# qq456cvb/CPPF2

Hardware: AMD Instinct MI355X
Metric: scenes/sec (1/2/4/8 GPU) at 4096 pts x 20k tuples; 5deg5cm match vs ref (higher is better)
Workload: dtype f32

## Files before the change

cppf2_amd/csrc/cppf_backvote.hip:

```cpp
#include "cppf_common.h"


template <typename KeyFn>
__device__ uint32_t radix_select_keys(KeyFn key, int n, int kth, uint32_t* s_hist , int* s_misc ,
                                      int* n_le) {
  uint32_t prefix = 0;
  int remaining = kth;
  int below = 0;
  const int shifts[3] = {21, 10, 0};
  const int widths[3] = {11, 11, 10};
  uint32_t mask_fixed = 0;
  for (int pass = 0; pass < 3; ++pass) {
    const int sh = shifts[pass], nbins = 1 << widths[pass];
    for (int i = threadIdx.x; i < nbins; i += blockDim.x) s_hist[i] = 0;
    __syncthreads();
    for (int i = threadIdx.x; i < n; i += blockDim.x) {
      const uint32_t bits = key(i);
      if ((bits & mask_fixed) == prefix) atomicAdd(&s_hist[(bits >> sh) & (nbins - 1)], 1u);
    }
    __syncthreads();
    if (threadIdx.x < 64) {
      const int per = nbins / 64;
      uint32_t sum = 0;
      for (int j = 0; j < per; ++j) sum += s_hist[threadIdx.x * per + j];
      uint32_t incl = sum;
#pragma unroll
      for (int off = 1; off < 64; off <<= 1) {
        const uint32_t o = __shfl_up(incl, off);
        if ((int)threadIdx.x >= off) incl += o;
      }
      const uint32_t excl = incl - sum;
      if ((uint32_t)remaining >= excl && (uint32_t)remaining < incl) {
        uint32_t run = excl;
        for (int j = 0; j < per; ++j) {
          const uint32_t c = s_hist[threadIdx.x * per + j];
          if ((uint32_t)remaining < run + c) {
            s_misc[0] = threadIdx.x * per + j;
            s_misc[1] = (int)run;
            s_misc[2] = (int)c;
            break;
          }
          run += c;
        }
      }
    }
    __syncthreads();
    const int bin = s_misc[0];
    below += s_misc[1];
    remaining -= s_misc[1];
    prefix |= ((uint32_t)bin) << sh;
    mask_fixed |= ((uint32_t)(nbins - 1)) << sh;
    if (pass == 2) *n_le = below + s_misc[2];
    __syncthreads();
  }
  return prefix;
}

__device__ uint32_t radix_select(const float* __restrict__ v, int n, int kth, uint32_t* s_hist, int* s_misc,
                                 int* n_le) {
  return radix_select_keys([v](int i) { return __float_as_uint(v[i]); }, n, kth, s_hist, s_misc, n_le);
}

__device__ __forceinline__ uint32_t float_key(float f) {
  const uint32_t u = __float_as_uint(f);
  return (u & 0x80000000u) ? ~u : (u | 0x80000000u);
}
__device__ __forceinline__ float key_float(uint32_t k) {
  return __uint_as_float((k & 0x80000000u) ? (k & 0x7fffffffu) : ~k);
}

__global__ __launch_bounds__(256) void backvote_errs_kernel(const float* __restrict__ pts,
                                                            const int32_t* __restrict__ pt_off,
                                                            const int32_t* __restrict__ idx, int k,
                                                            const int32_t* __restrict__ tup_off,
                                                            const float* __restrict__ tr,
                                                            const double* __restrict__ centers, Axes9 axes,
                                                            float* __restrict__ errs) {
  const int b = blockIdx.y;
  const float* p = pts + 3 * (int64_t)pt_off[b];
  const int t0 = tup_off[b], nt = tup_off[b + 1] - t0;
  const double cx = centers[3 * b], cy = centers[3 * b + 1], cz = centers[3 * b + 2];
  for (int t = blockIdx.x * 256 + threadIdx.x; t < nt; t += gridDim.x * 256) {
    const int64_t row = (int64_t)(t0 + t);
    const float* a = p + 3 * (int64_t)idx[row * k];
    const float* bb = p + 3 * (int64_t)idx[row * k + 1];
    float tb[2];
    target_pair(a[0], a[1], a[2], bb[0], bb[1], bb[2], cx, cy, cz, axes.a, tb, nullptr);
    const float d0 = tr[row * 2] - tb[0], d1 = tr[row * 2 + 1] - tb[1];
    errs[row] = __builtin_sqrtf(d0 * d0 + d1 * d1);
  }
}

__global__ __launch_bounds__(BV_THREADS) void backvote_kernel(
    const float* __restrict__ pts, const int32_t* __restrict__ pt_off, const int32_t* __restrict__ idx, int k,
    const int32_t* __restrict__ tup_off, const float* __restrict__ tr, const double* __restrict__ centers,
    Axes9 axes, const int32_t* __restrict__ kidx, const float* __restrict__ gammas, double margin, int num_rots,
    uint8_t* __restrict__ mask, int32_t* __restrict__ kept_tuple, int32_t* __restrict__ kept_count,
    double* __restrict__ kept_wt, int32_t* __restrict__ kept_row0, float* __restrict__ errs,
    float* __restrict__ thr_out, int32_t* __restrict__ hits) {
  __shared__ uint32_t s_hist[2048];
  __shared__ int s_misc[4];
  __shared__ int s_wave[BV_THREADS / 64];
  __shared__ float s_f[BV_THREADS / 64];
  const int b = blockIdx.x;
  const int p0 = pt_off[b];
  const float* p = pts + 3 * (int64_t)p0;
  const int t0 = tup_off[b], nt = tup_off[b + 1] - t0;
  float* e = errs + t0;
  if (nt <= 0) {
    if (threadIdx.x == 0) { kept_count[b] = 0; if (thr_out) thr_out[b] = NAN; }
    return;
  }
  int kq = kidx[b];
  if (kq > nt - 1) kq = nt - 1;
  const float gamma = gammas[b];
  int n_le = 0;
  const uint32_t bits_lo = radix_select(e, nt, kq, s_hist, s_misc, &n_le);
  const float v_lo = __uint_as_float(bits_lo);
  float v_hi = v_lo;
  if (kq + 1 <= nt - 1 && kq + 1 >= n_le) {
    uint32_t mn = 0xffffffffu;
    for (int i = threadIdx.x; i < nt; i += BV_THREADS) {
      const uint32_t bits = __float_as_uint(e[i]);
      if (bits > bits_lo && bits < mn) mn = bits;
    }
#pragma unroll
    for (int off = 32; off > 0; off >>= 1) mn = min(mn, (uint32_t)__shfl_xor((int)mn, off));
    if (wave_lane() == 0) s_hist[threadIdx.x >> 6] = mn;
    __syncthreads();
    if (threadIdx.x == 0) {
      for (int w = 1; w < BV_THREADS / 64; ++w) mn = min(mn, s_hist[w]);
      s_hist[64] = mn;
    }
    __syncthreads();
    v_hi = __uint_as_float(s_hist[64]);
    __syncthreads();
  }
  const float diff = v_hi - v_lo;
  float thr = v_lo + diff * gamma;
  if (gamma >= 0.5f) thr = v_hi - diff * (1.0f - gamma);
  if (threadIdx.x == 0 && thr_out) thr_out[b] = thr;
  int kept = 0;
  for (int base = 0; base < nt; base += BV_THREADS) {
    const int t = base + threadIdx.x;
    const bool keep = (t < nt) && (e[t] < thr);
    if (t < nt) mask[t0 + t] = keep ? 1 : 0;
    int tot;
    const int pos = block_scan_flag(keep, s_wave, &tot);
    if (keep) kept_tuple[t0 + kept + pos] = t;
    kept += tot;
  }
  if (threadIdx.x == 0) kept_count[b] = kept;
  __syncthreads();
  int32_t* h = hits + p0;
  for (int j = threadIdx.x; j < kept; j += BV_THREADS) {
    const int64_t row = (int64_t)(t0 + kept_tuple[t0 + j]);
    atomicAdd(&h[idx[row * k]], 1);
    atomicAdd(&h[idx[row * k + 1]], 1);
  }
  __threadfence();
  __syncthreads();
  int hmax = 0;
  for (int j = threadIdx.x; j < kept; j += BV_THREADS) {
    const int64_t row = (int64_t)(t0 + kept_tuple[t0 + j]);
    hmax = max(hmax, __hip_atomic_load(&h[idx[row * k]], __ATOMIC_RELAXED, __HIP_MEMORY_SCOPE_AGENT));
    hmax = max(hmax, __hip_atomic_load(&h[idx[row * k + 1]], __ATOMIC_RELAXED, __HIP_MEMORY_SCOPE_AGENT));
  }
#pragma unroll
  for (int off = 32; off > 0; off >>= 1) hmax = max(hmax, __shfl_xor(hmax, off));
  if (wave_lane() == 0) s_wave[threadIdx.x >> 6] = hmax;
  __syncthreads();
  hmax = 0;
  for (int w = 0; w < BV_THREADS / 64; ++w) hmax = max(hmax, s_wave[w]);
  __syncthreads();
  const double dmax = (double)hmax;
  int rank = 0;
  for (int base = 0; base < kept; base += BV_THREADS) {
    const int j = base + threadIdx.x;
    bool valid = false;
    if (j < kept) {
      const int64_t row = (int64_t)(t0 + kept_tuple[t0 + j]);
      const int i0 = idx[row * k], i1 = idx[row * k + 1];
      const double w0 = (double)__hip_atomic_load(&h[i0], __ATOMIC_RELAXED, __HIP_MEMORY_SCOPE_AGENT) / dmax;
      const double w1 = (double)__hip_atomic_load(&h[i1], __ATOMIC_RELAXED, __HIP_MEMORY_SCOPE_AGENT) / dmax;
      kept_wt[t0 + j] = (w0 + w1) + margin;
      const float dx = p[3 * i0] - p[3 * i1], dy = p[3 * i0 + 1] - p[3 * i1 + 1], dz = p[3 * i0 + 2] - p[3 * i1 + 2];
      valid = norm3_fused(dx, dy, dz) > 1e-7f;
    }
    int tot;
    const int pos = block_scan_flag(valid, s_wave, &tot);
    if (j < kept) kept_row0[t0 + j] = valid ? (rank + pos) * num_rots : -1;
    rank += tot;
  }
  (void)s_f;
}

extern "C" int64_t cppf_backvote_workspace_bytes(int64_t total_points, int B) {
  (void)B;
  return align_up(total_points * 4, 256);
}

extern "C" int cppf_backvote_filter(int B, const float* pts, const int32_t* pt_off, const int32_t* idx, int k,
                                    const int32_t* tup_off, const float* tr, const double* centers,
                                    const double* h_axes, const int32_t* kidx, const float* gammas,
                                    double imp_wt_margin, int num_rots, uint8_t* mask, int32_t* kept_tuple,
                                    int32_t* kept_count, double* kept_wt, int32_t* kept_row0, float* back_errs,
                                    float* thr, void* workspace, int64_t workspace_bytes, void* stream) {
  CPPF_CHECK_ARG(B > 0 && pts && pt_off && idx && tup_off && tr && centers && h_axes && kidx && gammas);
  CPPF_CHECK_ARG(mask && kept_tuple && kept_count && kept_wt && kept_row0 && back_errs);
  CPPF_CHECK_ARG(workspace && workspace_bytes > 0);
  Axes9 ax;
  for (int i = 0; i < 9; ++i) ax.a[i] = h_axes[i];
  CPPF_HIP(hipMemsetAsync(workspace, 0, (size_t)workspace_bytes, (hipStream_t)stream));
  hipLaunchKernelGGL(backvote_errs_kernel, dim3(B >= 32 ? 16 : 64, B), dim3(256), 0, (hipStream_t)stream, pts, pt_off,
                     idx, k, tup_off, tr, centers, ax, back_errs);
  CPPF_LAUNCH_CHECK();
  hipLaunchKernelGGL(backvote_kernel, dim3(B), dim3(BV_THREADS), 0, (hipStream_t)stream, pts, pt_off, idx, k, tup_off,
                     tr, centers, ax, kidx, gammas, imp_wt_margin, num_rots, mask, kept_tuple, kept_count, kept_wt,
                     kept_row0, back_errs, thr, (int32_t*)workspace);
  CPPF_LAUNCH_CHECK();
  return CPPF_OK;
}

#define ASM_STAGE 4096
__global__ __launch_bounds__(256) void assemble_pose_kernel(
    const float* __restrict__ sphere, const int32_t* __restrict__ up_idx, const float* __restrict__ up_count,
    const int32_t* __restrict__ right_idx, const float* __restrict__ right_count, int up_axis, int right_axis,
    const int64_t* __restrict__ argmax, const uint32_t* __restrict__ peak, const double* __restrict__ world,
    const CppfSceneGrid* __restrict__ grids, const float* __restrict__ pred_scales,
    const int32_t* __restrict__ tup_off, const int32_t* __restrict__ kept_tuple,
    const int32_t* __restrict__ kept_count, CppfSceneResult* __restrict__ out) {
  const int b = blockIdx.x;
  __shared__ float s_med[3];
  const int kept = kept_count ? kept_count[b] : 0;
  if (threadIdx.x < 3) s_med[threadIdx.x] = NAN;
  __syncthreads();
  if (pred_scales && kept > 0) {
    __shared__ uint32_t s_hist[2048];
    __shared__ int s_misc[4];
    const int t0 = tup_off[b];
    const int target = (kept - 1) / 2;
    __shared__ uint32_t s_keys[3][ASM_STAGE];
    const bool staged = kept <= ASM_STAGE;
    if (staged) {
      for (int i = threadIdx.x; i < kept; i += blockDim.x) {
        const float* row = pred_scales + (int64_t)(t0 + kept_tuple[t0 + i]) * 3;
        s_keys[0][i] = float_key(row[0]); s_keys[1][i] = float_key(row[1]); s_keys[2][i] = float_key(row[2]);
      }
      __syncthreads();
    }
    for (int col = 0; col < 3; ++col) {
      int n_le;
      uint32_t k;
      if (staged) {
        const uint32_t* keys = s_keys[col];
        k = radix_select_keys([=](int i) { return keys[i]; }, kept, target, s_hist, s_misc, &n_le);
      } else {
        k = radix_select_keys(
            [=](int i) { return float_key(pred_scales[(int64_t)(t0 + kept_tuple[t0 + i]) * 3 + col]); }, kept, target,
            s_hist, s_misc, &n_le);
      }
      if (threadIdx.x == 0) s_med[col] = key_float(k);
    }
  }
  __syncthreads();
  if (threadIdx.x != 0) return;
  CppfSceneResult r;
  r.argmax = argmax[b];
  r.peak = peak ? peak[b] : 0u;
  r.t[0] = world[3 * b]; r.t[1] = world[3 * b + 1]; r.t[2] = world[3 * b + 2];
  r.up_idx = up_idx[b]; r.right_idx = right_idx[b];
  r.up_count = up_count ? up_count[b] : 0.0f;
  r.right_count = right_count ? right_count[b] : 0.0f;
  r.kept = kept;
  r.flags = (grids ? grids[b].flags : 0) | ((peak && peak[b] == 0xFFFFFFFFu) ? 4 : 0);
  r.ncell = grids ? grids[b].ncell : 0;
  r.pad_[0] = r.pad_[1] = r.pad_[2] = 0;
  r.scale[0] = s_med[0]; r.scale[1] = s_med[1]; r.scale[2] = s_med[2];
  pose_from_bins(sphere, r.up_idx, r.right_idx, up_axis, right_axis, r.R);
  out[b] = r;
}

extern "C" int cppf_assemble_pose(int B, const float* sphere, const int32_t* up_idx, const float* up_count,
                                  const int32_t* right_idx, const float* right_count, int up_axis, int right_axis,
                                  const int64_t* argmax, const uint32_t* peak, const double* world,
                                  const CppfSceneGrid* grids, const float* pred_scales, const int32_t* tup_off,
                                  const int32_t* kept_tuple, const int32_t* kept_count, CppfSceneResult* out,
                                  void* stream) {
  CPPF_CHECK_ARG(B > 0 && sphere && up_idx && right_idx && argmax && world && out);
  CPPF_CHECK_ARG(up_axis >= 0 && up_axis < 3 && right_axis >= 0 && right_axis < 3 && up_axis != right_axis);
  CPPF_CHECK_ARG(pred_scales == nullptr || (tup_off && kept_tuple && kept_count));
  hipLaunchKernelGGL(assemble_pose_kernel, dim3(B), dim3(256), 0, (hipStream_t)stream, sphere, up_idx, up_count,
                     right_idx, right_count, up_axis, right_axis, argmax, peak, world, grids, pred_scales, tup_off,
                     kept_tuple, kept_count, out);
  CPPF_LAUNCH_CHECK();
  return CPPF_OK;
}

// ... 36 lines not shown
```

cppf2_amd/csrc/cppf_mlp_split.hip:

```cpp
#include "cppf_common.h"
#include <atomic>
#include <type_traits>

typedef float f32x16 __attribute__((ext_vector_type(16)));
typedef float f32x4 __attribute__((ext_vector_type(4)));
typedef __bf16 bf16x8 __attribute__((ext_vector_type(8)));

__host__ __device__ constexpr int rs_waves(int nt) { return nt >= 6 ? 4 : 8; }
#define RS_RESLAYER 0
#define RS_LINEAR 1
#define RS_SUMGATHER 2
#define RS_ENCODE 3
#define RS_SUMENCODE 5
__host__ __device__ constexpr int rs_waves_mode(int nt, int mode) { return mode == RS_LINEAR ? 8 : rs_waves(nt); }
#define RS_STAGE_TILES 16
#define RS_FRAG_BYTES 1024
__host__ __device__ constexpr int rs_stage_bytes(int stg) { return stg * 3 * RS_FRAG_BYTES; }
__host__ __device__ constexpr int rs_tile_bytes(int pc) { return pc * RS_FRAG_BYTES; }

#ifndef RS_DBG
#define RS_DBG 0
#endif
typedef unsigned u32x4 __attribute__((ext_vector_type(4)));
typedef float f32x2 __attribute__((ext_vector_type(2)));
// ... 229 lines not shown
  constexpr int SPC = rs_spc(NTILES, Stream::STG_);
  float xv[8];
  RS_WAIT(4, 15);
  __builtin_amdgcn_sched_barrier(0);
  xs.read(xv, 0, 0);
  RsFrag b = rs_split<PC>(xv);
  int slot = 1;
  bool whole = true;
  for (int s0 = 0; s0 < ks1; s0 += SPC) {
    const u32x4* w = (s0 > 0 && whole) ? ws.template acquire<2 * (SPC - 1)>() : ws.template acquire<0>();
    whole = s0 + SPC <= ks1;
#pragma unroll
    for (int i = 0; i < SPC; ++i) {
      if (s0 + i < ks1) {
        RS_WAIT(2, 15);
        __builtin_amdgcn_sched_barrier(0);
        xs.read(xv, s0 + i + 1, slot);
        xs.issue(s0 + i + 3, slot == 0 ? 2 : slot - 1, rw);
        slot = slot == 2 ? 0 : slot + 1;
        RsFrag bn;
        rs_step<NTILES, Stream::PMAX, PC>(acc, w + i * NTILES * PC * 64, b,
                        [&](int p) { rs_split_pair<PC, true>(xv[2 * p], xv[2 * p + 1], bn.h[p], bn.m[p], bn.l[p]); },
                        [&](int q) { if (i == 0) ws.piece(q); });
        b = bn;
      }
    }
  }
}

template <int NS, int NTILES, int PC, class Stream>
__device__ __forceinline__ void rs_product_h(f32x16 (&dst)[NTILES], const f32x16 (&src)[NS], Stream& ws, float bs) {
  constexpr int SPC = rs_spc(NTILES, Stream::STG_);
  static_assert((2 * NS) % SPC == 0, "whole chunks");
  RsFrag b;
#pragma unroll
  for (int p = 0; p < 4; ++p)
    rs_split_pair<PC>(PC == 2 ? src[0][2 * p] * bs : src[0][2 * p], PC == 2 ? src[0][2 * p + 1] * bs : src[0][2 * p + 1], b.h[p], b.m[p], b.l[p]);
#pragma unroll
  for (int c = 0; c < 2 * NS / SPC; ++c) {
    const u32x4* w = ws.template acquire<0>();
#pragma unroll
    for (int i = 0; i < SPC; ++i) {
      const int step = c * SPC + i, nx = (step + 1 < 2 * NS) ? step + 1 : step;
      RsFrag bn = b;
      rs_step<NTILES, Stream::PMAX, PC>(dst, w + i * NTILES * PC * 64, b,
                      [&](int p) {
                        if (step + 1 < 2 * NS) {
                          const float s0 = src[nx >> 1][8 * (nx & 1) + 2 * p], s1 = src[nx >> 1][8 * (nx & 1) + 2 * p + 1];
                          rs_split_pair<PC, true>(PC == 2 ? s0 * bs : s0, PC == 2 ? s1 * bs : s1, bn.h[p], bn.m[p], bn.l[p]);
                        }
                      },
                      [&](int q) { if (i == 0) ws.piece(q); });
      b = bn;
    }
  }
}

__device__ __forceinline__ float rs_relu(float h) { return __builtin_elementwise_maximum(h, 0.0f); }

__device__ __forceinline__ void rs_load_tile(f32x16& acc, const float* v, int g) {
#pragma unroll
  for (int q = 0; q < 4; ++q) {
    const f32x4 t = *reinterpret_cast<const f32x4*>(v + 8 * q + 4 * g);
    acc[4 * q + 0] = t.x; acc[4 * q + 1] = t.y; acc[4 * q + 2] = t.z; acc[4 * q + 3] = t.w;
  }
}

__device__ __forceinline__ void rs_load_tile_scaled(f32x16& acc, const float* v, int g, float sc) {
#pragma unroll
  for (int q = 0; q < 4; ++q) {
    const f32x4 t = *reinterpret_cast<const f32x4*>(v + 8 * q + 4 * g);
    acc[4 * q + 0] = t.x * sc; acc[4 * q + 1] = t.y * sc; acc[4 * q + 2] = t.z * sc; acc[4 * q + 3] = t.w * sc;
  }
}

struct RsDecode {
  const float* prior = nullptr;
  const float* prior_pos = nullptr;
  float prior_inv_sigma = 0.0f;
  const float* uniforms = nullptr;
  int32_t* bins = nullptr;
};

template <int NT, int PC>
__device__ __forceinline__ void rs_decode_epilogue(f32x16 (&o)[NT], const RsDecode& dc, int64_t row, bool in, int g, float bs) {
  static_assert(NT == 6, "6 coordinates x 32 bins");
  if (PC == 2) {
#pragma unroll
    for (int u = 0; u < 6; ++u) o[u] *= bs;
  }
  if (dc.prior) {
    const float* pr = dc.prior + row * 192 + 4 * g;
#pragma unroll
    for (int u = 0; u < 6; ++u) {
#pragma unroll
      for (int q = 0; q < 4; ++q) {
        const f32x4 v = *reinterpret_cast<const f32x4*>(pr + 32 * u + 8 * q);
        o[u][4 * q + 0] += v.x; o[u][4 * q + 1] += v.y; o[u][4 * q + 2] += v.z; o[u][4 * q + 3] += v.w;
      }
    }
  } else if (dc.prior_pos) {
    const float* pp = dc.prior_pos + row * 6;
    const float is = dc.prior_inv_sigma;
#pragma unroll
    for (int u = 0; u < 6; ++u) {
      const float pos = pp[u];
#pragma unroll
      for (int e = 0; e < 16; ++e) {
        const float z = ((float)((e & 3) + 8 * (e >> 2) + 4 * g) - pos) * is;
        o[u][e] += (z * z) * -0.5f;
      }
    }
  }
  float back[6], tot[6];
#pragma unroll
  for (int u = 0; u < 6; ++u) {
    float m = o[u][0];
#pragma unroll
    for (int e = 1; e < 16; ++e) m = fmaxf(m, o[u][e]);
    m = fmaxf(m, __shfl_xor(m, 32));
#pragma unroll
    for (int e = 0; e < 16; ++e) o[u][e] = softmax_exp(o[u][e] - m);
    back[u] = 0.0f;
  }
#pragma unroll
  for (int q = 0; q < 4; ++q) {
    float ta[6][4], tb[6][4], fwd[6];
#pragma unroll
    for (int u = 0; u < 6; ++u) {
      ta[u][0] = back[u] + o[u][4 * q + 0];
      ta[u][1] = ta[u][0] + o[u][4 * q + 1];
      ta[u][2] = ta[u][1] + o[u][4 * q + 2];
      ta[u][3] = ta[u][2] + o[u][4 * q + 3];
    }
#pragma unroll
    for (int u = 0; u < 6; ++u) fwd[u] = __shfl_xor(ta[u][3], 32);
#pragma unroll
    for (int u = 0; u < 6; ++u) {
      tb[u][0] = fwd[u] + o[u][4 * q + 0];
      tb[u][1] = tb[u][0] + o[u][4 * q + 1];
      tb[u][2] = tb[u][1] + o[u][4 * q + 2];
      tb[u][3] = tb[u][2] + o[u][4 * q + 3];
    }
#pragma unroll
    for (int u = 0; u < 6; ++u) {
      back[u] = __shfl_xor(tb[u][3], 32);
      tot[u] = g ? tb[u][3] : back[u];
#pragma unroll
      for (int i = 0; i < 4; ++i) o[u][4 * q + i] = g ? tb[u][i] : ta[u][i];
    }
  }
  const float* ur = dc.uniforms + row * 6;
#pragma unroll
  for (int u = 0; u < 6; ++u) {
    const float target = ur[u] * tot[u];
    int cnt = 0;
#pragma unroll
    for (int e = 0; e < 16; ++e) cnt += (o[u][e] <= target) ? 1 : 0;
    cnt += __shfl_xor(cnt, 32);
    if (in && g == 0) dc.bins[row * 6 + u] = cnt < 31 ? cnt : 31;
  }
}

__device__ __forceinline__ void rs_claim_store(int* p, int v) { __hip_atomic_store(p, v, __ATOMIC_RELAXED, __HIP_MEMORY_SCOPE_WORKGROUP); }
__device__ __forceinline__ int rs_claim_load(int* p) { return __hip_atomic_load(p, __ATOMIC_RELAXED, __HIP_MEMORY_SCOPE_WORKGROUP); }

struct RsTap {
  float* out = nullptr;
  int64_t ld = 0;
};

struct RsGather {
  const int32_t* gidx = nullptr;
  const float* table = nullptr;
  int slots = 0, head = 0, fshift = 0;
  int64_t tld = 0;
  const float* pts = nullptr;
  const float* nrm = nullptr;
  const int32_t* pt_off = nullptr;
  const int32_t* tup_off = nullptr;
  int B = 0;
  int* sched = nullptr;
};

struct RsRow3 {
  float x, y, z;
};

__device__ __forceinline__ void rs_encode_tiles(char* slots, int lane, int g, const float* __restrict__ pts, const float* __restrict__ nrm,
                                                const float* __restrict__ table, int fshift, int g0, int g1, int g2, int g3, int g4) {
  constexpr int PI_[10] = {0, 0, 0, 0, 1, 1, 1, 2, 2, 3}, PJ_[10] = {1, 2, 3, 4, 2, 3, 4, 3, 4, 4};
  const int gi[5] = {g0, g1, g2, g3, g4};
  float v[48];
  {
    float p[5][3];
#pragma unroll
    for (int q = 0; q < 5; ++q) {
      const RsRow3 r = *reinterpret_cast<const RsRow3*>(pts + 3 * (int64_t)gi[q]);
      p[q][0] = r.x; p[q][1] = r.y; p[q][2] = r.z;
    }
#pragma unroll
    for (int q = 0; q < 10; ++q)
#pragma unroll
      for (int c = 0; c < 3; ++c) v[3 * q + c] = p[PI_[q]][c] - p[PJ_[q]][c];
  }
  {
    float n[5][3];
#pragma unroll
    for (int q = 0; q < 5; ++q) {
      const RsRow3 r = *reinterpret_cast<const RsRow3*>(nrm + 3 * (int64_t)gi[q]);
      n[q][0] = r.x; n[q][1] = r.y; n[q][2] = r.z;
    }
#pragma unroll
    for (int q = 0; q < 10; ++q) {
      const float* ni = n[PI_[q]];
      const float* nj = n[PJ_[q]];
      const float s_ = (ni[0] * nj[0] + ni[1] * nj[1]) + ni[2] * nj[2];
      v[30 + q] = fmaxf(s_, -s_);
    }
  }
  {
    const float* d0 = table + ((int64_t)g0 << fshift);
    const f32x4 a = *reinterpret_cast<const f32x4*>(d0), b = *reinterpret_cast<const f32x4*>(d0 + 4);
    v[40] = a.x; v[41] = a.y; v[42] = a.z; v[43] = a.w; v[44] = b.x; v[45] = b.y; v[46] = b.z; v[47] = b.w;
  }
#pragma unroll
  for (int s = 0; s < 3; ++s) {
    f32x4 lo, hi;
    lo.x = g ? v[16 * s + 8] : v[16 * s + 0]; lo.y = g ? v[16 * s + 9] : v[16 * s + 1];
    lo.z = g ? v[16 * s + 10] : v[16 * s + 2]; lo.w = g ? v[16 * s + 11] : v[16 * s + 3];
    hi.x = g ? v[16 * s + 12] : v[16 * s + 4]; hi.y = g ? v[16 * s + 13] : v[16 * s + 5];
    hi.z = g ? v[16 * s + 14] : v[16 * s + 6]; hi.w = g ? v[16 * s + 15] : v[16 * s + 7];
    *reinterpret_cast<f32x4*>(slots + s * 2048 + lane * 16) = lo;
    *reinterpret_cast<f32x4*>(slots + s * 2048 + 1024 + lane * 16) = hi;
  }
}

__device__ __forceinline__ void rs_encode_coord_tiles(char* slots, int lane, int g, const float* __restrict__ pts, int g0, int g1, int g2,
                                                      int g3, int g4) {
  constexpr int PI_[10] = {0, 0, 0, 0, 1, 1, 1, 2, 2, 3}, PJ_[10] = {1, 2, 3, 4, 2, 3, 4, 3, 4, 4};
  const int gi[5] = {g0, g1, g2, g3, g4};
  float p[5][3], v[32];
// ... 634 lines not shown
```

cppf2_amd/csrc/cppf_vote_center.hip:

```cpp
#include "cppf_common.h"

#define VC_THREADS 1024
#ifndef VC_SLAB_CELLS
#define VC_SLAB_CELLS 36864
#endif
#define VC_ARG_BLOCKS 32
#ifndef VC_MAX_LDS_ROTS
#define VC_MAX_LDS_ROTS 512
#endif
#define VC_TAB_LEN (2 * VC_MAX_LDS_ROTS + 4)
#define VC_LDS_WORDS (VC_SLAB_CELLS + 2 * VC_TAB_LEN + (VC_THREADS / 64) * 64)
#ifndef VC_MIN_SLAB_CELLS
#define VC_MIN_SLAB_CELLS 8192
#endif
#ifndef VC_MIN_WAVES
#define VC_MIN_WAVES 4
#endif
#define VC_FRAME_FLOATS 12
#define VC_WT_SCALE 256.0f
#ifndef VC_QUANTUM
#define VC_QUANTUM 4
#endif
#ifndef VC_ARC_MARGIN
#define VC_ARC_MARGIN 0.02f
#endif

struct SlabBest {
  int64_t idx;
  uint32_t val;
  uint32_t pad;
};

struct VoteSetup {
  float cx, cy, cz, xx, xy, xz, yx, yy, yz;
  bool ok;
};

__device__ __forceinline__ VoteSetup vote_setup(const float* __restrict__ p, int i0, int i1, float proj, float od,
                                                float res) {
  VoteSetup s;
  const PairFrame f = pair_frame(p, i0, i1);
  s.ok = (f.nrm > 1e-7f) & (od > res);
  s.cx = f.ax - f.ux * proj; s.cy = f.ay - f.uy * proj; s.cz = f.az - f.uz * proj;
  s.xx = f.cox / f.nco * od; s.xy = f.coy / f.nco * od; s.xz = f.coz / f.nco * od;
  s.yx = cross_term(s.xy, f.uz, s.xz, f.uy);
  s.yy = cross_term(s.xz, f.ux, s.xx, f.uz);
  s.yz = cross_term(s.xx, f.uy, s.xy, f.ux);
  return s;
}

__device__ __forceinline__ int vote_cell(float cx, float cy, float cz, float xx, float xy, float xz, float yx,
                                         float yy, float yz, float cs, float sn, float c0x, float c0y, float c0z,
                                         float res, int gx, int gy, int gz) {
  const float ox = cs * xx + sn * yx;
  const float oy = cs * xy + sn * yy;
  const float oz = cs * xz + sn * yz;
  const float fx = ((cx + ox) - c0x) / res + 0.5f;
  const float fy = ((cy + oy) - c0y) / res + 0.5f;
  const float fz = ((cz + oz) - c0z) / res + 0.5f;
  const bool ok = (fx >= 1.0f) & (fy >= 1.0f) & (fz >= 1.0f) & (fx < (float)gx) & (fy < (float)gy) & (fz < (float)gz);
  if (!ok) return -1;
  return ((int)fx * gy + (int)fy) * gz + (int)fz;
}

__device__ __forceinline__ uint32_t vote_weight(const float* __restrict__ vote_wt, int64_t row) {
  if (!vote_wt) return 1u;
  const float w = fminf(fmaxf(vote_wt[row], 0.0f), 4.0f);
  return (uint32_t)(w * VC_WT_SCALE + 0.5f);
}

__global__ __launch_bounds__(256) void vote_frames_kernel(const float* __restrict__ pts,
                                                          const int32_t* __restrict__ pt_off,
                                                          const int32_t* __restrict__ idx, int k,
                                                          const int32_t* __restrict__ tup_off,
                                                          const float* __restrict__ tr,
                                                          const float* __restrict__ vote_wt, float res, int num_rots,
                                                          int64_t total, float* __restrict__ fr) {
  const int b = blockIdx.y;
  const float* p = pts + 3 * (int64_t)pt_off[b];
  const int t0 = tup_off[b], nt = tup_off[b + 1] - t0;
  const float kappa = (float)num_rots * 0.15915494309189535f;
  for (int t = blockIdx.x * blockDim.x + threadIdx.x; t < nt; t += gridDim.x * blockDim.x) {
    const int64_t row = (int64_t)(t0 + t);
    VoteSetup v = vote_setup(p, idx[row * k], idx[row * k + 1], tr[row * 2], tr[row * 2 + 1], res);
    if (!v.ok) v.cx = NAN;
    const float A = sqrtf(v.xx * v.xx + v.yx * v.yx);
    fr[0 * total + row] = v.cx; fr[1 * total + row] = v.cy; fr[2 * total + row] = v.cz;
    fr[3 * total + row] = v.xx; fr[4 * total + row] = v.xy; fr[5 * total + row] = v.xz;
    fr[6 * total + row] = v.yx; fr[7 * total + row] = v.yy; fr[8 * total + row] = v.yz;
    fr[9 * total + row] = (A > 1e-12f) ? 1.0f / A : 0.0f;
    fr[10 * total + row] = atan2f(v.yx, v.xx) * kappa;
    fr[11 * total + row] = __uint_as_float(vote_weight(vote_wt, row));
  }
}

struct ArcSet {
  int a0, n0, a1, n1;
};

__device__ __forceinline__ ArcSet slab_arcs(float cx, float invA, float phi, float c0x, float res, int xl, int xh,
                                            int num_rots) {
  ArcSet o;
  o.a0 = 0; o.n0 = 0; o.a1 = 0; o.n1 = 0;
  const float slop = 0.01f * res + 4e-7f * (fabsf(cx) + fabsf(c0x));
  const float L = ((float)xl - 0.5f) * res + c0x - cx - slop;
  const float U = ((float)xh + 0.5f) * res + c0x - cx + slop;
  if (!(L <= U)) return o;
  if (invA == 0.0f) {
    if (L <= 0.0f && 0.0f <= U) o.n0 = num_rots;
    return o;
  }
  const float cl = L * invA - 1e-6f, cu = U * invA + 1e-6f;
  if (cl > 1.0f || cu < -1.0f) return o;
  const float kappa = (float)num_rots * 0.15915494309189535f;
  const float amin = acosf(fminf(cu, 1.0f)) * kappa;
  const float amax = acosf(fmaxf(cl, -1.0f)) * kappa;
  const float half = 0.5f * (float)num_rots;
  const bool near_merge = amin <= 0.5f;
  const bool far_merge = (half - amax) <= 0.5f;
  if (near_merge && far_merge) { o.n0 = num_rots; return o; }
  int b0;
  if (near_merge) {
    o.a0 = (int)ceilf(phi - amax - VC_ARC_MARGIN); b0 = (int)floorf(phi + amax + VC_ARC_MARGIN);
  } else if (far_merge) {
    o.a0 = (int)ceilf(phi + amin - VC_ARC_MARGIN); b0 = (int)floorf(phi + (float)num_rots - amin + VC_ARC_MARGIN);
  } else {
    o.a0 = (int)ceilf(phi + amin - VC_ARC_MARGIN); b0 = (int)floorf(phi + amax + VC_ARC_MARGIN);
    o.a1 = (int)ceilf(phi - amax - VC_ARC_MARGIN);
    o.n1 = max((int)floorf(phi - amin + VC_ARC_MARGIN) - o.a1 + 1, 0);
  }
  o.n0 = max(b0 - o.a0 + 1, 0);
  if (o.n0 >= num_rots) { o.a0 = 0; o.n0 = num_rots; o.n1 = 0; }
  return o;
}

#define VC_DPP(x, ctrl, rmask) __builtin_amdgcn_update_dpp(0, (x), (ctrl), (rmask), 0xf, false)
__device__ __forceinline__ int wave_incl_scan_add(int x) {
  x += VC_DPP(x, 0x111, 0xf);
  x += VC_DPP(x, 0x112, 0xf);
  x += VC_DPP(x, 0x114, 0xf);
  x += VC_DPP(x, 0x118, 0xf);
  x += VC_DPP(x, 0x142, 0xa);
  x += VC_DPP(x, 0x143, 0xc);
  return x;
}
__device__ __forceinline__ int wave_incl_scan_max(int x) {
  x = max(x, VC_DPP(x, 0x111, 0xf));
  x = max(x, VC_DPP(x, 0x112, 0xf));
  x = max(x, VC_DPP(x, 0x114, 0xf));
  x = max(x, VC_DPP(x, 0x118, 0xf));
  x = max(x, VC_DPP(x, 0x142, 0xa));
  x = max(x, VC_DPP(x, 0x143, 0xc));
  return x;
}

typedef float vc_f2 __attribute__((ext_vector_type(2)));

struct GridFast {
  float c0x, c0y, c0z, rinv;
  float lo_m, hi_m;
  int gx, gy, gz;
};

__device__ __forceinline__ vc_f2 vc_pk_fma(vc_f2 a, vc_f2 b, vc_f2 c) {
  vc_f2 d;
// ... 244 lines not shown
      if (c) atomicAdd(&pp[i], c);
    }
    __syncthreads();
    if (threadIdx.x == 0) {
      __threadfence();
      s_ticket = atomicAdd(&tickets[(int64_t)b * s_max + s], 1);
      __threadfence();
    }
    __syncthreads();
    if (s_ticket != Pl - 1) return;
    for (int i = threadIdx.x; i < n; i += VC_THREADS)
      slab[i] = __hip_atomic_load(&pp[i], __ATOMIC_RELAXED, __HIP_MEMORY_SCOPE_AGENT);
    __syncthreads();
  }
  const int64_t goff = grid ? (grid_off ? grid_off[b] : (int64_t)b * cells_cap) : 0;
  if (P == 1) {
    uint32_t bv = 0;
    int64_t bi = INT64_MAX;
    for (int i = threadIdx.x; i < n; i += VC_THREADS) {
      const uint32_t c = slab[i];
      if (grid) grid[goff + lo + i] = c;
      argmax_combine(bv, bi, c, (int64_t)(lo + i));
    }
    wave_argmax(bv, bi);
    __shared__ uint32_t s_v[VC_THREADS / 64];
    __shared__ int64_t s_i[VC_THREADS / 64];
    if (wave_lane() == 0) { s_v[threadIdx.x >> 6] = bv; s_i[threadIdx.x >> 6] = bi; }
    __syncthreads();
    if (threadIdx.x == 0) {
      for (int w = 1; w < VC_THREADS / 64; ++w) argmax_combine(bv, bi, s_v[w], s_i[w]);
      SlabBest o; o.idx = bi; o.val = bv;
      o.pad = 0;
#ifdef VC_DIAG
      o.pad = (uint32_t)(wall_clock64() - t_start);
      if (VC_DIAG == 1) o.pad = (uint32_t)(t_a - t_start);
      if (VC_DIAG == 2) o.pad = (uint32_t)(t_b - t_a);
      if (VC_DIAG == 3) o.pad = (uint32_t)(wall_clock64() - t_b);
      if (VC_DIAG == 4) o.pad = (uint32_t)nwin * 100;
#endif
      slab_best[(int64_t)b * s_max + s] = o;
    }
  } else {
    for (int i = threadIdx.x; i < n; i += VC_THREADS) {
      const uint32_t c = slab[i];
      if (c) atomicAdd(&grid[goff + lo + i], c);
    }
  }
}


__device__ __forceinline__ void vote_stage_tables(uint32_t* slab, int num_rots, const float* __restrict__ cos_tab,
                                                  const float* __restrict__ sin_tab) {
  float* s_cos = reinterpret_cast<float*>(slab + VC_SLAB_CELLS);
  float* s_sin = s_cos + VC_TAB_LEN;
  for (int i = threadIdx.x; i < 2 * num_rots + 4; i += VC_THREADS) {
    const int r = i % num_rots;
    s_cos[i] = cos_tab[r];
    s_sin[i] = sin_tab[r];
  }
  slab[VC_SLAB_CELLS + 2 * VC_TAB_LEN + threadIdx.x] = 0u;
}

template <bool ARCS, bool WEIGHTED>
__global__ __launch_bounds__(VC_THREADS, VC_MIN_WAVES) void vote_center_slab_kernel(
    const float* __restrict__ fr, int64_t total, const int32_t* __restrict__ tup_off, float res, int num_rots,
    const float* __restrict__ cos_tab, const float* __restrict__ sin_tab, const CppfSceneGrid* __restrict__ grids,
    uint32_t* __restrict__ grid, const int64_t* __restrict__ grid_off, int64_t cells_cap,
    SlabBest* __restrict__ slab_best, int s_max, int P) {
  extern __shared__ __attribute__((aligned(16))) uint32_t slab[];
  int tag = 0;
  const int pc = blockIdx.y, rank = blockIdx.z;
  const int b = (blockIdx.x + rank) % gridDim.x;
  const CppfSceneGrid g = grids[b];
  const int G = ((int64_t)g.ncell <= cells_cap) ? g.ncell : 0;
  const int nslab = (G + VC_SLAB_CELLS - 1) / VC_SLAB_CELLS;
  if (rank >= nslab) return;
  const int mid = nslab >> 1, dd = (rank + 1) >> 1;
  const int s = (rank & 1) ? mid - dd : mid + dd;
  if (ARCS) vote_stage_tables(slab, num_rots, cos_tab, sin_tab);
  vote_slab_item<ARCS, WEIGHTED>(slab, tag, b, s, VC_SLAB_CELLS, pc, P, g, G, fr, total, tup_off, res, num_rots, cos_tab, sin_tab,
                                 grid, grid_off, cells_cap, slab_best, s_max, P, nullptr, nullptr);
}

__global__ __launch_bounds__(1024) void vote_worklist_kernel(const CppfSceneGrid* __restrict__ grids, int B,
                                                             int64_t cells_cap, int s_max, int max_parts, int target,
                                                             uint32_t* __restrict__ list, int* __restrict__ ctl) {
  __shared__ int s_wave[16];
  __shared__ int s_base, s_maxg, s_cells;
  __shared__ unsigned long long s_sumg;
  if (threadIdx.x == 0) { s_base = 0; s_maxg = 0; s_sumg = 0ull; }
  __syncthreads();
  int mx = 0;
  unsigned long long sm = 0ull;
  for (int b = threadIdx.x; b < B; b += 1024) {
    const int G = ((int64_t)grids[b].ncell <= cells_cap) ? grids[b].ncell : 0;
    mx = max(mx, G);
    sm += (unsigned long long)G;
  }
  if (mx > 0) { atomicMax(&s_maxg, mx); atomicAdd(&s_sumg, sm); }
  __syncthreads();
  if (threadIdx.x == 0) {
    int64_t sc = max_parts > 1 ? (int64_t)VC_SLAB_CELLS : ((int64_t)s_sumg + target - 1) / max(target, 1);
    sc = max(sc, (int64_t)VC_MIN_SLAB_CELLS);
    sc = max(sc, ((int64_t)s_maxg + s_max - 1) / max(s_max, 1));
    sc = (sc + 255) / 256 * 256;
    s_cells = (int)min(sc, (int64_t)VC_SLAB_CELLS);
  }
  __syncthreads();
  const int slab_cells = s_cells;
  const int s_maxn = (s_maxg + slab_cells - 1) / slab_cells;
  const int64_t cand = (int64_t)B * min(s_maxn, s_max);
  for (int64_t base = 0; base < cand; base += 1024) {
    const int64_t c = base + threadIdx.x;
    int cnt = 0, b = 0, s = 0;
    if (c < cand) {
      const int rank = (int)(c / B), x = (int)(c % B);
      b = (x + rank) % B;
      const int G = ((int64_t)grids[b].ncell <= cells_cap) ? grids[b].ncell : 0;
      const int nslab = (G + slab_cells - 1) / slab_cells;
      if (rank < nslab) {
        cnt = 1;
        const int mid = nslab >> 1, dd = (rank + 1) >> 1;
        s = (rank & 1) ? mid - dd : mid + dd;
      }
    }
    const int incl = wave_incl_scan_add(cnt);
    if (wave_lane() == 63) s_wave[threadIdx.x >> 6] = incl;
    __syncthreads();
    int off = s_base;
    for (int w = 0; w < (int)(threadIdx.x >> 6); ++w) off += s_wave[w];
    off += incl - cnt;
    if (cnt) list[off] = (uint32_t)b | ((uint32_t)s << 16);
    __syncthreads();
    if (threadIdx.x == 1023) s_base = off + cnt;
    __syncthreads();
  }
  if (threadIdx.x == 0) {
    const int items = s_base;
    int P = 1;
    if (max_parts > 1 && items > 0 && items < target) P = min(max_parts, (target + items - 1) / items);
    ctl[0] = 0; ctl[1] = items * P; ctl[2] = P;
    ctl[3] = slab_cells;
  }
}

template <bool WEIGHTED>
__global__ __launch_bounds__(VC_THREADS, VC_MIN_WAVES) void vote_center_persist_kernel(
    const float* __restrict__ fr, int64_t total, const int32_t* __restrict__ tup_off, float res, int num_rots,
    const float* __restrict__ cos_tab, const float* __restrict__ sin_tab, const CppfSceneGrid* __restrict__ grids,
    uint32_t* __restrict__ grid, const int64_t* __restrict__ grid_off, int64_t cells_cap,
    SlabBest* __restrict__ slab_best, int s_max, const uint32_t* __restrict__ list, int* __restrict__ ctl,
    uint32_t* __restrict__ part, int* __restrict__ tickets) {
  extern __shared__ __attribute__((aligned(16))) uint32_t slab[];
  __shared__ int s_item;
  int tag = 0;
  vote_stage_tables(slab, num_rots, cos_tab, sin_tab);
  const int count = ctl[1], parts = ctl[2], slab_cells = ctl[3];
  for (;;) {
    __syncthreads();
    if (threadIdx.x == 0) s_item = atomicAdd(&ctl[0], 1);
    __syncthreads();
    const int item = s_item;
    if (item >= count) break;
    const uint32_t e = list[item / parts];
    const int b = (int)(e & 0xffffu), s = (int)(e >> 16);
    const CppfSceneGrid g = grids[b];
    vote_slab_item<true, WEIGHTED>(slab, tag, b, s, slab_cells, item % parts, parts, g, g.ncell, fr, total, tup_off, res, num_rots,
                                   cos_tab, sin_tab, grid, grid_off, cells_cap, slab_best, s_max, 1, part, tickets);
  }
}

__global__ __launch_bounds__(256) void vote_center_global_kernel(
    const float* __restrict__ pts, const int32_t* __restrict__ pt_off, const int32_t* __restrict__ idx, int k,
    const int32_t* __restrict__ tup_off, const float* __restrict__ tr, const float* __restrict__ vote_wt, float res,
    int num_rots, const float* __restrict__ cos_tab, const float* __restrict__ sin_tab,
    const CppfSceneGrid* __restrict__ grids, uint32_t* __restrict__ grid, const int64_t* __restrict__ grid_off,
    int64_t cells_cap) {
  const int b = blockIdx.y;
  const CppfSceneGrid g = grids[b];
  if ((int64_t)g.ncell > cells_cap || g.ncell <= 0) return;
  const float* p = pts + 3 * (int64_t)pt_off[b];
  const int t0 = tup_off[b], nt = tup_off[b + 1] - t0;
  uint32_t* gb = grid + (grid_off ? grid_off[b] : (int64_t)b * cells_cap);
  for (int t = blockIdx.x * blockDim.x + threadIdx.x; t < nt; t += gridDim.x * blockDim.x) {
    const int64_t row = (int64_t)(t0 + t);
    const VoteSetup v = vote_setup(p, idx[row * k], idx[row * k + 1], tr[row * 2], tr[row * 2 + 1], res);
    if (!v.ok) continue;
    const uint32_t wv = vote_weight(vote_wt, row);
    for (int r = 0; r < num_rots; ++r) {
      const int lin = vote_cell(v.cx, v.cy, v.cz, v.xx, v.xy, v.xz, v.yx, v.yy, v.yz, cos_tab[r], sin_tab[r],
                                g.c0[0], g.c0[1], g.c0[2], res, g.g[0], g.g[1], g.g[2]);
      if (lin >= 0) atomicAdd(&gb[lin], wv);
    }
  }
}

__global__ __launch_bounds__(256) void grid_argmax_partial_kernel(const uint32_t* __restrict__ grid,
                                                                  const int64_t* __restrict__ grid_off,
                                                                  int64_t cells_cap,
                                                                  const CppfSceneGrid* __restrict__ grids,
                                                                  SlabBest* __restrict__ partial, int s_max) {
  const int b = blockIdx.y;
  const int G = ((int64_t)grids[b].ncell <= cells_cap) ? grids[b].ncell : 0;
  const uint32_t* gb = grid + (grid_off ? grid_off[b] : (int64_t)b * cells_cap);
  const int per = (G + gridDim.x - 1) / gridDim.x;
  const int lo = blockIdx.x * per, hi = min(G, lo + per);
  uint32_t bv = 0;
  int64_t bi = INT64_MAX;
  for (int i = lo + threadIdx.x; i < hi; i += blockDim.x) argmax_combine(bv, bi, gb[i], (int64_t)i);
  wave_argmax(bv, bi);
  __shared__ uint32_t s_v[4];
  __shared__ int64_t s_i[4];
  if (wave_lane() == 0) { s_v[threadIdx.x >> 6] = bv; s_i[threadIdx.x >> 6] = bi; }
  __syncthreads();
  if (threadIdx.x == 0) {
    for (int w = 1; w < 4; ++w) argmax_combine(bv, bi, s_v[w], s_i[w]);
    SlabBest o; o.idx = bi; o.val = bv; o.pad = 0;
// ... 177 lines not shown
  L.best = 0;
  L.ctl = L.best + align_up(parts * (int64_t)sizeof(SlabBest), 256);
  L.list = L.ctl + 256;
  L.tickets = L.ctl + align_up(parts * 4 + 256, 256);
  L.grid = L.tickets + align_up(parts * 4, 256);
  L.frames = L.grid + align_up((int64_t)B * cells_cap * 4, 256);
  L.bytes = L.frames + align_up(total_tuples * VC_FRAME_FLOATS * 4, 256);
  return L;
}

extern "C" int64_t cppf_vote_center_workspace_bytes(int B, int64_t cells_cap, int64_t total_tuples) {
  if (B <= 0 || cells_cap <= 0 || total_tuples < 0) return 0;
  return vc_layout(B, cells_cap, total_tuples).bytes;
}

constexpr int VC_MODE_NO_PERSIST = 0x800;

enum VcPath { VC_PERSIST, VC_SLAB, VC_GLOBAL };

struct VcPlan {
  VcPath path;
  bool arcs, weighted, prepare, vote;
  int P, max_parts, s_max, s_max_parts;
};

static int vc_plan(int mode, int B, int max_t, int num_rots, int64_t cells_cap, bool weighted, VcPlan* p) {
  const int s_max = (int)((cells_cap + VC_SLAB_CELLS - 1) / VC_SLAB_CELLS);
  int m = mode & 0xff;
  if (m == 0) m = (s_max <= 64) ? 1 : 2;
  if (max_t <= 0) m = 2;
  if (m < 1 || m > 3) {
    snprintf(g_cppf_err, sizeof(g_cppf_err), "cppf_vote_center: unknown mode %d", m);
    return CPPF_EINVAL;
  }
  const bool arcs = m == 1 && s_max > 1 && num_rots <= VC_MAX_LDS_ROTS && num_rots >= 8;
  const bool persist = arcs && B <= 0xffff && s_max <= 0xffff && !(mode & VC_MODE_NO_PERSIST);
  *p = VcPlan{m == 2 ? VC_GLOBAL : persist ? VC_PERSIST : VC_SLAB, arcs, weighted, m == 2 || !(mode & CPPF_VC_FRAMES_READY),
              m == 2 || !(mode & CPPF_VC_FRAMES_ONLY), 1, 1, s_max, vc_parts(cells_cap)};
  const int pmax_t = (max_t + VC_THREADS - 1) / VC_THREADS;
  const int64_t wgs = (int64_t)B * s_max;
  if (persist && B <= 48) p->max_parts = std::min(pmax_t, 64);
  if (p->path == VC_SLAB && wgs < 256) p->P = (int)std::min<int64_t>((256 + wgs - 1) / wgs, pmax_t);
  return CPPF_OK;
}

extern "C" int cppf_vote_center(int B, const float* pts, const int32_t* pt_off, const int32_t* idx, int k,
                                const int32_t* tup_off, int max_t, int64_t total_tuples, const float* tr,
                                const float* vote_wt, double res, int num_rots, const float* cos_tab, const float* sin_tab, const CppfSceneGrid* grids,
                                uint32_t* grid, const int64_t* grid_off, int64_t cells_cap, int mode,
                                void* workspace, int64_t workspace_bytes, int64_t* out_argmax, uint32_t* out_peak,
                                double* out_world, void* stream) {
  CPPF_CHECK_ARG(B > 0 && pts && pt_off && idx && tup_off && tr && cos_tab && sin_tab && grids && out_argmax);
  CPPF_CHECK_ARG(k >= 2 && num_rots > 0 && res > 0.0 && cells_cap > 0 && cells_cap <= 0x7fffffffLL);
  CPPF_CHECK_ARG(total_tuples >= 0 && max_t >= 0 && (int64_t)max_t <= total_tuples);
  const VcLayout L = vc_layout(B, cells_cap, total_tuples);
  CPPF_CHECK_ARG(workspace && workspace_bytes >= L.bytes);
  CPPF_CHECK_ARG(grid == nullptr || grid_off != nullptr);
  VcPlan p;
  CPPF_TRY(vc_plan(mode, B, max_t, num_rots, cells_cap, vote_wt != nullptr, &p));
  hipStream_t st = (hipStream_t)stream;
  char* ws = (char*)workspace;
  SlabBest* best = (SlabBest*)(ws + L.best);
  int *ctl = (int*)(ws + L.ctl), *tickets = (int*)(ws + L.tickets);
  uint32_t *list = (uint32_t*)(ws + L.list), *ws_grid = (uint32_t*)(ws + L.grid);
  float* frames = (float*)(ws + L.frames);
  const float res32 = (float)res;
  const int lds_bytes = VC_LDS_WORDS * 4;
  int dev = 0, num_cus = 0;
  if (p.path != VC_GLOBAL) {
    CPPF_TRY(cppf_device_cus(&dev, &num_cus));
    const void* fns[] = {(const void*)vote_center_slab_kernel<true, false>, (const void*)vote_center_slab_kernel<true, true>,
                         (const void*)vote_center_slab_kernel<false, false>, (const void*)vote_center_slab_kernel<false, true>,
                         (const void*)vote_center_persist_kernel<false>, (const void*)vote_center_persist_kernel<true>};
    for (const void* f : fns) CPPF_TRY(cppf_allow_dynamic_lds(f, dev, lds_bytes));
  }
  const bool merge = p.path == VC_GLOBAL || p.P > 1;
  uint32_t* target = (merge && !grid) ? ws_grid : grid;
  const int64_t* target_off = (merge && !grid) ? nullptr : grid_off;
  if (merge) {
    hipLaunchKernelGGL(grid_zero_kernel, dim3(64, B), dim3(256), 0, st, target, target_off, cells_cap, grids);
    CPPF_LAUNCH_CHECK();
  }
  if (p.prepare && p.path != VC_GLOBAL) {
    hipLaunchKernelGGL(vote_frames_kernel, dim3((max_t + 255) / 256, B), dim3(256), 0, st, pts, pt_off, idx, k, tup_off, tr, vote_wt,
                       res32, num_rots, total_tuples, frames);
    if (p.path == VC_PERSIST) {
      hipLaunchKernelGGL(vote_worklist_kernel, dim3(1), dim3(1024), 0, st, grids, B, cells_cap, p.s_max_parts, p.max_parts,
                         2 * num_cus, list, ctl);
      if (p.max_parts > 1) {
        hipLaunchKernelGGL(grid_zero_kernel, dim3(64, B), dim3(256), 0, st, ws_grid, (const int64_t*)nullptr, cells_cap, grids);
        CPPF_HIP(hipMemsetAsync(tickets, 0, (size_t)B * p.s_max_parts * 4, st));
      }
    }
    CPPF_LAUNCH_CHECK();
  }
  if (!p.vote) return CPPF_OK;
  if (p.path == VC_PERSIST)
    hipLaunchKernelGGL((p.weighted ? vote_center_persist_kernel<true> : vote_center_persist_kernel<false>), dim3(num_cus),
                       dim3(VC_THREADS), lds_bytes, st, frames, total_tuples, tup_off, res32, num_rots, cos_tab, sin_tab, grids, grid,
                       grid_off, cells_cap, best, p.s_max_parts, list, ctl, p.max_parts > 1 ? ws_grid : nullptr, tickets);
  else if (p.path == VC_SLAB)
    hipLaunchKernelGGL((p.arcs ? (p.weighted ? vote_center_slab_kernel<true, true> : vote_center_slab_kernel<true, false>)
                               : (p.weighted ? vote_center_slab_kernel<false, true> : vote_center_slab_kernel<false, false>)),
                       dim3(B, p.P, p.s_max), dim3(VC_THREADS), lds_bytes, st, frames, total_tuples, tup_off, res32, num_rots, cos_tab,
                       sin_tab, grids, target, target_off, cells_cap, best, p.s_max_parts, p.P);
  else if (max_t > 0)
    hipLaunchKernelGGL(vote_center_global_kernel, dim3((max_t + 255) / 256, B), dim3(256), 0, st, pts, pt_off, idx, k, tup_off, tr,
                       vote_wt, res32, num_rots, cos_tab, sin_tab, grids, target, target_off, cells_cap);
  CPPF_LAUNCH_CHECK();
  if (merge)
    hipLaunchKernelGGL(grid_argmax_partial_kernel, dim3(VC_ARG_BLOCKS, B), dim3(256), 0, st, target, target_off, cells_cap, grids,
                       best, p.s_max_parts);
  hipLaunchKernelGGL(grid_argmax_final_kernel, dim3(B), dim3(64), 0, st, best, p.s_max_parts, merge ? VC_ARG_BLOCKS : 0,
                     p.path == VC_PERSIST ? ctl : nullptr, grids, cells_cap, res, out_argmax, out_peak, out_world);
  CPPF_LAUNCH_CHECK();
  return CPPF_OK;
}

extern "C" int64_t cppf_grid_peaks_workspace_bytes(int B, int K) {
  if (B <= 0 || K < 1 || K > GP_MAX_K) return 0;
  return align_up((int64_t)B * K * 8, 256);
}

extern "C" int cppf_grid_peaks(int B, const CppfSceneGrid* grids, const uint32_t* grid, const int64_t* grid_off,
                               int64_t cells_cap, double res, int K, int sep_cells, int64_t* peak_idx, uint32_t* peak_val,
                               double* peak_world, int32_t* n_peaks, void* workspace, int64_t workspace_bytes, void* stream) {
  CPPF_CHECK_ARG(B > 0 && B <= 0xffff && grids && grid && peak_idx);
  CPPF_CHECK_ARG(K >= 1 && K <= GP_MAX_K && sep_cells >= 0 && res > 0.0 && cells_cap > 0 && cells_cap <= 0x7fffffffLL);
  const int64_t need = cppf_grid_peaks_workspace_bytes(B, K);
  CPPF_CHECK_ARG(workspace && workspace_bytes >= need);
  hipStream_t st = (hipStream_t)stream;
  unsigned long long* keys = (unsigned long long*)workspace;
  CPPF_HIP(hipMemsetAsync(keys, 0, (size_t)B * K * 8, st));
  int nbx = (int)std::min<int64_t>(std::max<int64_t>((cells_cap + GP_THREADS * 16 - 1) / (GP_THREADS * 16), 1), 256);
  if ((int64_t)nbx * B > 8192) nbx = std::max(1, 8192 / B);
  const long long sep2 = (long long)sep_cells * sep_cells;
  for (int k = 0; k < K; ++k)
    hipLaunchKernelGGL(grid_peaks_pass_kernel, dim3(nbx, B), dim3(GP_THREADS), 0, st, grid, grid_off, cells_cap, grids, keys, K, k,
                       sep2);
  hipLaunchKernelGGL(grid_peaks_final_kernel, dim3(B), dim3(64), 0, st, keys, K, grids, cells_cap, res, peak_idx, peak_val,
                     peak_world, n_peaks);
  CPPF_LAUNCH_CHECK();
  return CPPF_OK;
}
```

Before: 6134.

## Fold memsets and worklist launch into kernels; use permlane32 swaps in decode

The backvote workspace memset is replaced by zeroing the per-point hit counters inside the error kernel. The vote worklist kernel and the tickets memset are folded into an extra block of the frames kernel, which removes separate launches and memset calls from the stream. In the MLP decode epilogue, cross-half wave shuffles (__shfl_xor by 32) become permlane32_swap builtins, which avoid LDS-based shuffles. The risks are that the workspace memset previously cleared the whole workspace and not just the point range, and that the worklist now runs with 256 threads instead of 1024.

```diff
diff --git a/cppf2_amd/csrc/cppf_backvote.hip b/cppf2_amd/csrc/cppf_backvote.hip
--- a/cppf2_amd/csrc/cppf_backvote.hip
+++ b/cppf2_amd/csrc/cppf_backvote.hip
@@ -75,8 +75,9 @@
                                                             const int32_t* __restrict__ tup_off,
                                                             const float* __restrict__ tr,
                                                             const double* __restrict__ centers, Axes9 axes,
-                                                            float* __restrict__ errs) {
+                                                            float* __restrict__ errs, int32_t* __restrict__ hits) {
   const int b = blockIdx.y;
+  for (int i = pt_off[b] + blockIdx.x * 256 + threadIdx.x; i < pt_off[b + 1]; i += gridDim.x * 256) hits[i] = 0;
   const float* p = pts + 3 * (int64_t)pt_off[b];
   const int t0 = tup_off[b], nt = tup_off[b + 1] - t0;
   const double cx = centers[3 * b], cy = centers[3 * b + 1], cz = centers[3 * b + 2];
@@ -211,9 +212,8 @@
   CPPF_CHECK_ARG(workspace && workspace_bytes > 0);
   Axes9 ax;
   for (int i = 0; i < 9; ++i) ax.a[i] = h_axes[i];
-  CPPF_HIP(hipMemsetAsync(workspace, 0, (size_t)workspace_bytes, (hipStream_t)stream));
   hipLaunchKernelGGL(backvote_errs_kernel, dim3(B >= 32 ? 16 : 64, B), dim3(256), 0, (hipStream_t)stream, pts, pt_off,
-                     idx, k, tup_off, tr, centers, ax, back_errs);
+                     idx, k, tup_off, tr, centers, ax, back_errs, (int32_t*)workspace);
   CPPF_LAUNCH_CHECK();
   hipLaunchKernelGGL(backvote_kernel, dim3(B), dim3(BV_THREADS), 0, (hipStream_t)stream, pts, pt_off, idx, k, tup_off,
                      tr, centers, ax, kidx, gammas, imp_wt_margin, num_rots, mask, kept_tuple, kept_count, kept_wt,
diff --git a/cppf2_amd/csrc/cppf_mlp_split.hip b/cppf2_amd/csrc/cppf_mlp_split.hip
--- a/cppf2_amd/csrc/cppf_mlp_split.hip
+++ b/cppf2_amd/csrc/cppf_mlp_split.hip
@@ -335,6 +335,13 @@
   int32_t* bins = nullptr;
 };
 
+__device__ __forceinline__ float rs_lower_to_both(float v) {
+  return __uint_as_float(__builtin_amdgcn_permlane32_swap(__float_as_uint(v), __float_as_uint(v), false, false)[0]);
+}
+__device__ __forceinline__ float rs_upper_to_lower(float v, float spare) {
+  return __uint_as_float(__builtin_amdgcn_permlane32_swap(__float_as_uint(v), __float_as_uint(spare), false, false)[1]);
+}
+
 template <int NT, int PC>
 __device__ __forceinline__ void rs_decode_epilogue(f32x16 (&o)[NT], const RsDecode& dc, int64_t row, bool in, int g, float bs) {
   static_assert(NT == 6, "6 coordinates x 32 bins");
@@ -371,14 +378,17 @@
     float m = o[u][0];
 #pragma unroll
     for (int e = 1; e < 16; ++e) m = fmaxf(m, o[u][e]);
-    m = fmaxf(m, __shfl_xor(m, 32));
+    {
+      const auto h = __builtin_amdgcn_permlane32_swap(__float_as_uint(m), __float_as_uint(m), false, false);
+      m = fmaxf(__uint_as_float(h[0]), __uint_as_float(h[1]));
+    }
 #pragma unroll
     for (int e = 0; e < 16; ++e) o[u][e] = softmax_exp(o[u][e] - m);
     back[u] = 0.0f;
   }
 #pragma unroll
   for (int q = 0; q < 4; ++q) {
-    float ta[6][4], tb[6][4], fwd[6];
+    float ta[6][4], tb[6][4];
 #pragma unroll
     for (int u = 0; u < 6; ++u) {
       ta[u][0] = back[u] + o[u][4 * q + 0];
@@ -387,22 +397,23 @@
       ta[u][3] = ta[u][2] + o[u][4 * q + 3];
     }
 #pragma unroll
-    for (int u = 0; u < 6; ++u) fwd[u] = __shfl_xor(ta[u][3], 32);
+    for (int u = 0; u < 6; ++u) ta[u][3] = rs_lower_to_both(ta[u][3]);
 #pragma unroll
     for (int u = 0; u < 6; ++u) {
-      tb[u][0] = fwd[u] + o[u][4 * q + 0];
+      tb[u][0] = ta[u][3] + o[u][4 * q + 0];
       tb[u][1] = tb[u][0] + o[u][4 * q + 1];
       tb[u][2] = tb[u][1] + o[u][4 * q + 2];
       tb[u][3] = tb[u][2] + o[u][4 * q + 3];
     }
 #pragma unroll
     for (int u = 0; u < 6; ++u) {
-      back[u] = __shfl_xor(tb[u][3], 32);
-      tot[u] = g ? tb[u][3] : back[u];
 #pragma unroll
       for (int i = 0; i < 4; ++i) o[u][4 * q + i] = g ? tb[u][i] : ta[u][i];
-    }
-  }
+      back[u] = rs_upper_to_lower(tb[u][3], ta[u][3]);
+    }
+  }
+#pragma unroll
+  for (int u = 0; u < 6; ++u) tot[u] = g ? o[u][15] : back[u];
   const float* ur = dc.uniforms + row * 6;
 #pragma unroll
   for (int u = 0; u < 6; ++u) {
@@ -410,7 +421,10 @@
     int cnt = 0;
 #pragma unroll
     for (int e = 0; e < 16; ++e) cnt += (o[u][e] <= target) ? 1 : 0;
-    cnt += __shfl_xor(cnt, 32);
+    {
+      const auto h = __builtin_amdgcn_permlane32_swap((unsigned)cnt, (unsigned)cnt, false, false);
+      cnt = (int)(h[0] + h[1]);
+    }
     if (in && g == 0) dc.bins[row * 6 + u] = cnt < 31 ? cnt : 31;
   }
 }
diff --git a/cppf2_amd/csrc/cppf_vote_center.hip b/cppf2_amd/csrc/cppf_vote_center.hip
--- a/cppf2_amd/csrc/cppf_vote_center.hip
+++ b/cppf2_amd/csrc/cppf_vote_center.hip
@@ -69,18 +69,34 @@
   return (uint32_t)(w * VC_WT_SCALE + 0.5f);
 }
 
+struct VoteWork {
+  const CppfSceneGrid* grids;
+  int64_t cells_cap;
+  int s_max, max_parts, target;
+  uint32_t* list;
+  int* ctl;
+  int* tickets;
+};
+template <int THREADS>
+__device__ void vote_worklist(const VoteWork& w, int B);
+
 __global__ __launch_bounds__(256) void vote_frames_kernel(const float* __restrict__ pts,
                                                           const int32_t* __restrict__ pt_off,
                                                           const int32_t* __restrict__ idx, int k,
                                                           const int32_t* __restrict__ tup_off,
                                                           const float* __restrict__ tr,
                                                           const float* __restrict__ vote_wt, float res, int num_rots,
-                                                          int64_t total, float* __restrict__ fr) {
+                                                          int64_t total, float* __restrict__ fr, VoteWork work) {
   const int b = blockIdx.y;
+  const int frame_blocks = (int)gridDim.x - (work.list ? 1 : 0);
+  if ((int)blockIdx.x == frame_blocks) {
+    if (b == 0) vote_worklist<256>(work, (int)gridDim.y);
+    return;
+  }
   const float* p = pts + 3 * (int64_t)pt_off[b];
   const int t0 = tup_off[b], nt = tup_off[b + 1] - t0;
   const float kappa = (float)num_rots * 0.15915494309189535f;
-  for (int t = blockIdx.x * blockDim.x + threadIdx.x; t < nt; t += gridDim.x * blockDim.x) {
+  for (int t = blockIdx.x * blockDim.x + threadIdx.x; t < nt; t += frame_blocks * blockDim.x) {
     const int64_t row = (int64_t)(t0 + t);
     VoteSetup v = vote_setup(p, idx[row * k], idx[row * k + 1], tr[row * 2], tr[row * 2 + 1], res);
     if (!v.ok) v.cx = NAN;
@@ -491,17 +507,23 @@
                                  grid, grid_off, cells_cap, slab_best, s_max, P, nullptr, nullptr);
 }
 
-__global__ __launch_bounds__(1024) void vote_worklist_kernel(const CppfSceneGrid* __restrict__ grids, int B,
-                                                             int64_t cells_cap, int s_max, int max_parts, int target,
-                                                             uint32_t* __restrict__ list, int* __restrict__ ctl) {
-  __shared__ int s_wave[16];
+template <int THREADS>
+__device__ void vote_worklist(const VoteWork& w, int B) {
+  const CppfSceneGrid* __restrict__ grids = w.grids;
+  const int64_t cells_cap = w.cells_cap;
+  const int s_max = w.s_max, max_parts = w.max_parts, target = w.target;
+  uint32_t* __restrict__ list = w.list;
+  int* __restrict__ ctl = w.ctl;
+  __shared__ int s_wave[THREADS / 64];
   __shared__ int s_base, s_maxg, s_cells;
   __shared__ unsigned long long s_sumg;
   if (threadIdx.x == 0) { s_base = 0; s_maxg = 0; s_sumg = 0ull; }
   __syncthreads();
+  if (max_parts > 1)
+    for (int64_t i = threadIdx.x; i < (int64_t)B * s_max; i += THREADS) w.tickets[i] = 0;
   int mx = 0;
   unsigned long long sm = 0ull;
-  for (int b = threadIdx.x; b < B; b += 1024) {
+  for (int b = threadIdx.x; b < B; b += THREADS) {
     const int G = ((int64_t)grids[b].ncell <= cells_cap) ? grids[b].ncell : 0;
     mx = max(mx, G);
     sm += (unsigned long long)G;
@@ -519,7 +541,7 @@
   const int slab_cells = s_cells;
   const int s_maxn = (s_maxg + slab_cells - 1) / slab_cells;
   const int64_t cand = (int64_t)B * min(s_maxn, s_max);
-  for (int64_t base = 0; base < cand; base += 1024) {
+  for (int64_t base = 0; base < cand; base += THREADS) {
     const int64_t c = base + threadIdx.x;
     int cnt = 0, b = 0, s = 0;
     if (c < cand) {
@@ -537,11 +559,11 @@
     if (wave_lane() == 63) s_wave[threadIdx.x >> 6] = incl;
     __syncthreads();
     int off = s_base;
-    for (int w = 0; w < (int)(threadIdx.x >> 6); ++w) off += s_wave[w];
+    for (int wv = 0; wv < (int)(threadIdx.x >> 6); ++wv) off += s_wave[wv];
     off += incl - cnt;
     if (cnt) list[off] = (uint32_t)b | ((uint32_t)s << 16);
     __syncthreads();
-    if (threadIdx.x == 1023) s_base = off + cnt;
+    if (threadIdx.x == THREADS - 1) s_base = off + cnt;
     __syncthreads();
   }
   if (threadIdx.x == 0) {
@@ -885,16 +907,12 @@
     CPPF_LAUNCH_CHECK();
   }
   if (p.prepare && p.path != VC_GLOBAL) {
-    hipLaunchKernelGGL(vote_frames_kernel, dim3((max_t + 255) / 256, B), dim3(256), 0, st, pts, pt_off, idx, k, tup_off, tr, vote_wt,
-                       res32, num_rots, total_tuples, frames);
-    if (p.path == VC_PERSIST) {
-      hipLaunchKernelGGL(vote_worklist_kernel, dim3(1), dim3(1024), 0, st, grids, B, cells_cap, p.s_max_parts, p.max_parts,
-                         2 * num_cus, list, ctl);
-      if (p.max_parts > 1) {
-        hipLaunchKernelGGL(grid_zero_kernel, dim3(64, B), dim3(256), 0, st, ws_grid, (const int64_t*)nullptr, cells_cap, grids);
-        CPPF_HIP(hipMemsetAsync(tickets, 0, (size_t)B * p.s_max_parts * 4, st));
-      }
-    }
+    const bool persist = p.path == VC_PERSIST;
+    const VoteWork work = {grids, cells_cap, p.s_max_parts, p.max_parts, 2 * num_cus, persist ? list : nullptr, ctl, tickets};
+    hipLaunchKernelGGL(vote_frames_kernel, dim3((max_t + 255) / 256 + (persist ? 1 : 0), B), dim3(256), 0, st, pts, pt_off, idx, k,
+                       tup_off, tr, vote_wt, res32, num_rots, total_tuples, frames, work);
+    if (persist && p.max_parts > 1)
+      hipLaunchKernelGGL(grid_zero_kernel, dim3(64, B), dim3(256), 0, st, ws_grid, (const int64_t*)nullptr, cells_cap, grids);
     CPPF_LAUNCH_CHECK();
   }
   if (!p.vote) return CPPF_OK;
```

After: 6128. About the same (-0.1%).
